# taha-kms/CLASSMATE-RAG

Hardware: AMD Instinct MI355X
Metric: hybrid queries/sec + recall@10 vs reference, 10M×768 chunks, 1/2/4/8 GPU (higher is better)
Workload: dtype fp32-accurate E5 (K10 f16x3 MFMA) + int8/f16/f64 dense + f64 BM25

## Files before the change

classmate-rag_amd/csrc/cm_dense_q8.inc:

```

#ifndef K1Q_RING
#define K1Q_RING 12
#endif
#ifndef K1Q_DBG
#define K1Q_DBG 0
#endif
constexpr int kQDbg = K1Q_DBG;
constexpr int kQRing = K1Q_RING;
constexpr int kQCap = 128;
#ifndef K1Q_RR
#define K1Q_RR 4096
#endif
#ifndef K1Q_RT
#define K1Q_RT 1024
#endif
constexpr int kQBand = K1Q_RR;
constexpr int kQBand2 = K1Q_RR / 2;
constexpr int kQRT = K1Q_RT, kQRW = K1Q_RT / 64;
constexpr int kQSel = 256;
constexpr int kQMeta = 4;
#ifndef K1Q_LDS
#define K1Q_LDS (160 * 1024)
#endif
#ifndef K1Q_LDS_SHARED
#define K1Q_LDS_SHARED (131 * 1024)
#endif
constexpr int q8_vm_after(int y, int z) {
  int n = 2 * (z - y);
  for (int x = y; x <= z; ++x) n += x % 6 == 0 ? 1 : 0;
  return n;
}

typedef int i32x4q __attribute__((ext_vector_type(4)));

__host__ __device__ inline void q8_ge(int k6, int &g, int &e) {
  g = k6 >> 4;
  e = k6 & 15;
}
__host__ __device__ inline int64_t q8_plane_off(int64_t row, int k, int ld) {
  const int64_t tile = row >> 6;
  const int rr = (int)(row & 63), rt = rr >> 4, j = rr & 15;
  const int c = k >> 7, kk = k & 127, kh = kk >> 6;
  int g, e;
  q8_ge(kk & 63, g, e);
  return (((tile * (ld >> 7) + c) * 8 + rt * 2 + kh) << 10) + ((g * 16 + j) << 4) + e;
}
__host__ __device__ inline int64_t q8_query_off(int64_t q, int k, int ld) {
  const int64_t qt = q >> 4;
  const int j = (int)(q & 15);
  const int c = k >> 7, kk = k & 127, kh = kk >> 6;
  int g, e;
  q8_ge(kk & 63, g, e);
  return (((qt * (ld >> 7) + c) * 2 + kh) << 10) + ((g * 16 + j) << 4) + e;
}

__device__ inline float block256_max(float v, float *red) {
  for (int o = 32; o > 0; o >>= 1) v = fmaxf(v, __shfl_xor(v, o));
  __syncthreads();
  if ((threadIdx.x & 63) == 0) red[threadIdx.x >> 6] = v;
  __syncthreads();
  return fmaxf(fmaxf(red[0], red[1]), fmaxf(red[2], red[3]));
}
__device__ inline double block256_sum(double v, double *red) {
  for (int o = 32; o > 0; o >>= 1) v += __shfl_xor(v, o);
  __syncthreads();
  if ((threadIdx.x & 63) == 0) red[threadIdx.x >> 6] = v;
  __syncthreads();
  return (red[0] + red[1]) + (red[2] + red[3]);
}

template <typename XN, typename PUT>
__device__ inline float3 q8_quantise(XN xn_of, PUT put, int ld) {
  __shared__ float redf[4];
  __shared__ double redd[4];
  float amax = 0.f;
  for (int c = threadIdx.x; c < ld; c += 256) amax = fmaxf(amax, fabsf(xn_of(c)));
  amax = block256_max(amax, redf);
  const float s = amax > 0.f ? amax / 127.f : 1.f;
  double er = 0.0, nr = 0.0;
  for (int c = threadIdx.x; c < ld; c += 256) {
    const float x = xn_of(c);
    const int q = max(-127, min(127, (int)rintf(x / s)));
    put(c, (int8_t)q);
    const double xt = (double)s * (double)q;
    er += ((double)x - xt) * ((double)x - xt);
    nr += xt * xt;
  }
  er = block256_sum(er, redd);
  nr = block256_sum(nr, redd);
  return make_float3(s, (float)(sqrt(er) * (1.0 + 1e-6)), (float)(sqrt(nr) * (1.0 + 1e-6)));
}

__host__ __device__ inline int64_t q8_group_of(int64_t row) { return (row >> 6) * 4 + ((row >> 2) & 3); }
__host__ __device__ inline int64_t q8_group_row(int64_t G, int i) {
  return (G >> 2) * 64 + 16 * (i >> 2) + 4 * (G & 3) + (i & 3);
}
__global__ void __launch_bounds__(256) dense_q8_group_kernel(const float *__restrict__ C, const float *__restrict__ invc,
                                                             const int64_t *__restrict__ groups, int64_t g0, int64_t ng,
                                                             int dim, int ld, int8_t *__restrict__ Xq,
                                                             float2 *__restrict__ rmeta, uint32_t *__restrict__ rnorm) {
  const int64_t gi = blockIdx.x;
  if (gi >= ng) return;
  const int64_t G = groups ? groups[gi] : g0 + gi;
  const int i = threadIdx.x >> 4, l = threadIdx.x & 15;
  const int64_t r = q8_group_row(G, i);
  const float inv = invc[r];
  const float *crow = C + r * ld;
  auto xn_of = [&](int c) { return c < dim ? crow[c] * inv : 0.f; };
  __shared__ float redf[4];
  float amax = 0.f;
  for (int c = l; c < ld; c += 16) amax = fmaxf(amax, fabsf(xn_of(c)));
  amax = block256_max(amax, redf);
  const float s = amax > 0.f ? amax / 127.f : 1.f;
  double er = 0.0, nr = 0.0;
  for (int c = l; c < ld; c += 16) {
    const float x = xn_of(c);
    const int q = max(-127, min(127, (int)rintf(x / s)));
    Xq[q8_plane_off(r, c, ld)] = (int8_t)q;
    const double xt = (double)s * (double)q;
    er += ((double)x - xt) * ((double)x - xt);
    nr += xt * xt;
  }
  for (int o = 8; o > 0; o >>= 1) {
    er += __shfl_xor(er, o);
    nr += __shfl_xor(nr, o);
  }
  if (l == 0) {
    rmeta[r] = make_float2(s, (float)(sqrt(er) * (1.0 + 1e-6)));
    atomicMax(&rnorm[2], __float_as_uint((float)(sqrt(nr) * (1.0 + 1e-6))));
  }
}

__global__ void __launch_bounds__(256) dense_prep_q8(const float *__restrict__ q, int nq, int dim, int ld,
                                                     int8_t *__restrict__ Qq, float4 *__restrict__ qsc,
                                                     const uint32_t *__restrict__ rnorm) {
  const int qi = blockIdx.x;
  const float *src = q + (int64_t)qi * dim;
  __shared__ double redd[4];
  double t = 0.0;
  float tf = 0.f;
  for (int i = threadIdx.x; i < dim; i += 256) {
    const float v = qi < nq ? src[i] : 0.f;
    tf += v * v;
  }
  __shared__ float redf[4];
  for (int o = 32; o > 0; o >>= 1) tf += __shfl_xor(tf, o);
  if ((threadIdx.x & 63) == 0) redf[threadIdx.x >> 6] = tf;
  __syncthreads();
  const float tt = (redf[0] + redf[1]) + (redf[2] + redf[3]);
  const float inv = 1.0f / (sqrtf(tt) + 1e-30f);
  auto xn_of = [&](int c) { return (qi < nq && c < dim) ? src[c] * inv : 0.f; };
  const float3 m = q8_quantise(xn_of, [&](int c, int8_t v) { Qq[q8_query_off(qi, c, ld)] = v; }, ld);
  for (int c = threadIdx.x; c < ld; c += 256) {
    const double x = (double)xn_of(c);
    t += x * x;
  }
  t = block256_sum(t, redd);
  if (threadIdx.x == 0) {
    const double nmax = (double)__uint_as_float(rnorm[2]);
    const float a = (float)(nmax * (double)m.y * (1.0 + 1e-6) + 4e-6);
    const float b = (float)(sqrt(t) * (1.0 + 1e-6));
    qsc[qi] = make_float4(m.x, a, b, sqrtf(tt));
  }
}

constexpr int kQDumpB = 96;
#ifndef K1Q_RING_FULL
#define K1Q_RING_FULL K1Q_RING
#endif
template <int LDS>
struct K1qLds {
  static constexpr int ring = LDS >= 160 * 1024 ? K1Q_RING_FULL : kQRing;
  static constexpr int stage_e = (LDS - ring * 8192 - kQMeta * 1024 - 1024) / (4 * kQDumpB);
  static constexpr int cnt_off = ring * 8192 + kQMeta * 1024 + 4 * stage_e * kQDumpB;
  static constexpr int total = cnt_off + 1024;
  static_assert(total <= 160 * 1024 && stage_e >= 64, "K1q LDS: ring + metadata + staging + counters");
};
constexpr int kQLds = K1qLds<K1Q_LDS>::total, kQLdsShared = K1qLds<K1Q_LDS_SHARED>::total;
template <int LDS = K1Q_LDS>
__global__ void __launch_bounds__(256, 1)
    dense_q8_scan_kernel(const int8_t *__restrict__ Xq, const float2 *__restrict__ rmeta,
                         const uint32_t *__restrict__ live, const uint32_t *__restrict__ allow, int64_t n_words,
                         const int8_t *__restrict__ Qq, const float4 *__restrict__ qsc, int nq,
                         const float *__restrict__ seed, int64_t rows_per_wg, int64_t rows_end, int n_wg,
                         uint64_t *__restrict__ out_keys, float *__restrict__ out_up,
                         uint32_t *__restrict__ out_cnt) {
  constexpr int KC = 6, QT = 4, PCS = 2, RING = K1qLds<LDS>::ring;
  constexpr int kQStageE = K1qLds<LDS>::stage_e, kQCntOff = K1qLds<LDS>::cnt_off;
  static_assert(RING > KC + 1, "the tile's row scales must be younger than every chunk the tile waits for");
  extern __shared__ __attribute__((aligned(16))) unsigned char lds[];
  const int tid = threadIdx.x, lane = tid & 63, g = lane >> 4, j = lane & 15;
  const int wave = __builtin_amdgcn_readfirstlane(tid >> 6);
  const int wg = blockIdx.x % n_wg, qp = blockIdx.x / n_wg;
  const int64_t r_begin = (int64_t)wg * rows_per_wg;
  const int64_t r_end = min(r_begin + rows_per_wg, rows_end);
  const int ntiles = r_begin < r_end ? (int)((r_end - r_begin) >> 6) : 0;
  const int total = ntiles * KC;
  const int qc0 = wave * 64;
  const int64_t qt0 = ((int64_t)qp * kBQPass + qc0) >> 4;
  i32x4q qf[KC][2][QT];
#pragma unroll
  for (int c = 0; c < KC; ++c)
#pragma unroll
    for (int kh = 0; kh < 2; ++kh)
#pragma unroll
      for (int qt = 0; qt < QT; ++qt)
        qf[c][kh][qt] = *reinterpret_cast<const i32x4q *>(Qq + ((((qt0 + qt) * KC + c) * 2 + kh) << 10) + lane * 16);
#pragma unroll
  for (int c = 0; c < KC; ++c)
#pragma unroll
    for (int kh = 0; kh < 2; ++kh)
#pragma unroll
      for (int qt = 0; qt < QT; ++qt) asm volatile("" : "+a"(qf[c][kh][qt]));
  float sq[QT], oaq[QT], aq[QT], bq[QT], sdq[QT];
#pragma unroll
  for (int qt = 0; qt < QT; ++qt) {
    const int qq = qp * kBQPass + qc0 + qt * 16 + j;
    const float4 v = qsc[qq];
    sq[qt] = v.x;
    aq[qt] = v.y;
    oaq[qt] = 1.0f - v.y;
    bq[qt] = v.z;
    sdq[qt] = qq < nq ? seed[qq] : -__builtin_inff();
  }
  __builtin_amdgcn_s_waitcnt(0x0F70);
  const __attribute__((address_space(1))) unsigned char *Xb = (const __attribute__((address_space(1))) unsigned char *)Xq;
  const int64_t cb = (r_begin >> 6) * KC;
  const uint32_t *allw = allow ? allow : live;
  unsigned char *meta = lds + RING * 8192;
  auto issue_meta = [&](int T) __attribute__((always_inline)) {
    const int Tc = min(T, ntiles - 1);
    const int64_t row0 = r_begin + (int64_t)Tc * 64;
    const unsigned char *src;
    if (wave == 2) {
      const int64_t wi = (row0 >> 5) + (lane & 1);
      const int64_t wc = wi < n_words ? wi : n_words - 1;
      src = reinterpret_cast<const unsigned char *>((lane & 2) ? allw + wc : live + wc);
    } else {
      src = reinterpret_cast<const unsigned char *>(rmeta + row0) + (wave & 1) * 256 + lane * 4;
    }
    __builtin_amdgcn_global_load_lds((const __attribute__((address_space(1))) void *)src,
                                     (__attribute__((address_space(3))) void *)(meta + (T % kQMeta) * 1024 + wave * 256),
                                     4, 0, 0);
  };
  auto issue_piece = [&](int gc, int i) __attribute__((always_inline)) {
    int gl = min(gc, total - 1);
    if (kQDbg & 8192) gl &= 15;
    const int o = 4 * i + wave;
    __builtin_amdgcn_global_load_lds(Xb + (((cb + gl) * 8 + o) << 10) + lane * 16,
                                     (__attribute__((address_space(3))) void *)(lds + (gc % RING) * 8192 + o * 1024),
                                     16, 0, kK1cAux);
  };
  auto issue = [&](int gc, bool tile_start) __attribute__((always_inline)) {
#pragma unroll
    for (int i = 0; i < PCS; ++i) issue_piece(gc, i);
    if (tile_start) issue_meta(gc / KC);
  };
  auto frag = [&](int gc, int rt, int kh) -> i32x4q {
    return *reinterpret_cast<const i32x4q *>(lds + (gc % RING) * 8192 + (rt * 2 + kh) * 1024 + lane * 16);
  };
  const uint32_t stg = (uint32_t)(uintptr_t)(const __attribute__((address_space(3))) unsigned char *)(
      lds + RING * 8192 + kQMeta * 1024 + wave * kQStageE * kQDumpB);
  const uint32_t cnt_lds = (uint32_t)(uintptr_t)(const __attribute__((address_space(3))) unsigned char *)(
      lds + kQCntOff + wave * 256);
  const int64_t qbuf0 = ((int64_t)qp * n_wg + wg) * kBQPass + qc0;
  uint32_t nst = 0, dbg_sink = 0;
  auto process = [&](uint32_t n) __attribute__((always_inline)) -> uint32_t {
    if (kQDbg & 16) return 0u;
    for (uint32_t e = lane; e < n; e += 64) {
      const uint32_t a0 = stg + e * kQDumpB;
      i32x4q h0, h1, av0, av1, av2, av3;
      asm volatile("ds_read_b128 %0, %6\n\t"
                   "ds_read_b128 %1, %6 offset:16\n\t"
                   "ds_read_b128 %2, %6 offset:32\n\t"
                   "ds_read_b128 %3, %6 offset:48\n\t"
                   "ds_read_b128 %4, %6 offset:64\n\t"
                   "ds_read_b128 %5, %6 offset:80\n\t"
                   "s_waitcnt lgkmcnt(0)"
                   : "=&v"(h0), "=&v"(h1), "=&v"(av0), "=&v"(av1), "=&v"(av2), "=&v"(av3)
                   : "v"(a0)
                   : "memory");
      const uint32_t ql = (uint32_t)h0[0] & 63u, live16 = (uint32_t)h0[0] >> 16;
      const int64_t rb = (int64_t)(uint32_t)h0[1];
      const float A = __int_as_float(h0[2]), B = __int_as_float(h0[3]);
      const float W = __int_as_float(h1[0]), sd = __int_as_float(h1[1]);
      const i32x4q av[4] = {av0, av1, av2, av3};
      uint32_t hm = 0;
#pragma unroll
      for (int i = 0; i < 16; ++i)
        hm |= (fmaf(-A, (float)av[i >> 2][i & 3], B) <= sd ? 1u : 0u) << i;
      hm &= live16;
      uint32_t slot;
      asm volatile("ds_add_rtn_u32 %0, %1, %2\n\ts_waitcnt lgkmcnt(0)"
                   : "=v"(slot) : "v"(cnt_lds + ql * 4), "v"((kQDbg & (2 | 32)) ? 0u : (uint32_t)__popc(hm))
                   : "memory");
      const int64_t ob = (qbuf0 + ql) * kQCap;
      if (kQDbg & 32) hm = 0;
      while (hm) {
        const int i = __builtin_ctz(hm);
        hm &= hm - 1u;
        int av_i;
        asm volatile("ds_read_b32 %0, %1\n\ts_waitcnt lgkmcnt(0)" : "=v"(av_i) : "v"(a0 + 32 + 4 * i) : "memory");
        if (slot < (uint32_t)kQCap && !(kQDbg & 2)) {
          const float lo = fmaf(-A, (float)av_i, B);
          const int64_t row = rb + 16 * (i >> 2) + (i & 3);
          out_keys[ob + slot] = ((uint64_t)f32_order(lo) << 32) | (uint64_t)(uint32_t)row;
          out_up[ob + slot] = lo + W;
        }
        ++slot;
      }
    }
    return 0u;
  };
  reinterpret_cast<uint32_t *>(lds + kQCntOff)[tid] = 0u;
  i32x4q acc[4][QT];
#pragma unroll
  for (int rt = 0; rt < 4; ++rt)
#pragma unroll
    for (int qt = 0; qt < QT; ++qt) acc[rt][qt] = i32x4q{0, 0, 0, 0};

  if (total > 0) {
#pragma unroll
    for (int p = 0; p < RING; ++p) issue(p, p % KC == 0);
    asm volatile("s_waitcnt vmcnt(%0)" ::"n"(q8_vm_after(0, RING - 1)) : "memory");
    __builtin_amdgcn_s_barrier();
    i32x4q xf[4][2];
#pragma unroll
    for (int rt = 0; rt < 2; ++rt)
#pragma unroll
      for (int kh = 0; kh < 2; ++kh) xf[rt][kh] = frag(0, rt, kh);
    constexpr int W0 = 16 - PCS - 2;
    const uint32_t meta_lds = (uint32_t)(uintptr_t)(const __attribute__((address_space(3))) unsigned char *)meta;
    int pm[QT];
    uint32_t eu = 0u, s_bits = 0u;
    i32x4q wdv;
    uint64_t ev[8];
    auto tail = [&](int m, int t) __attribute__((always_inline)) {
      const uint32_t mb = meta_lds + (t % kQMeta) * 1024;
      if (m == 0) {
        asm volatile("ds_read_b128 %0, %10 offset:512\n\t"
                     "ds_read_b32 %1, %11\n\t"
                     "ds_read2_b32 %2, %11 offset0:1 offset1:3\n\t"
                     "ds_read2_b32 %3, %11 offset0:5 offset1:7\n\t"
                     "ds_read2_b32 %4, %11 offset0:33 offset1:35\n\t"
                     "ds_read2_b32 %5, %11 offset0:37 offset1:39\n\t"
                     "ds_read2_b32 %6, %11 offset0:65 offset1:67\n\t"
                     "ds_read2_b32 %7, %11 offset0:69 offset1:71\n\t"
                     "ds_read2_b32 %8, %11 offset0:97 offset1:99\n\t"
                     "ds_read2_b32 %9, %11 offset0:101 offset1:103"
                     : "=&v"(wdv), "=&v"(s_bits), "=&v"(ev[0]), "=&v"(ev[1]), "=&v"(ev[2]), "=&v"(ev[3]),
                       "=&v"(ev[4]), "=&v"(ev[5]), "=&v"(ev[6]), "=&v"(ev[7])
                     : "v"(mb), "v"(mb + 32 * g)
                     : "memory");
      }
      if (m >= 3 && m <= 10) {
        const int q = (m - 3) >> 1;
        if (((m - 3) & 1) == 0) {
          pm[q] = max(max(acc[0][q][0], acc[0][q][1]), acc[0][q][2]);
          pm[q] = max(max(pm[q], acc[0][q][3]), acc[1][q][0]);
        } else {
          pm[q] = max(max(pm[q], acc[1][q][1]), acc[1][q][2]);
          pm[q] = max(pm[q], acc[1][q][3]);
        }
        asm volatile("" : "+v"(pm[q]));
      }
      if (m == 11) asm volatile("s_waitcnt lgkmcnt(0)" ::: "memory");
      if (m >= 11 && m <= 14) {
        const int k0 = 2 * (m - 11);
        eu = max(max(m == 11 ? 0u : eu, (uint32_t)ev[k0]), (uint32_t)(ev[k0] >> 32));
        eu = max(max(eu, (uint32_t)ev[k0 + 1]), (uint32_t)(ev[k0 + 1] >> 32));
        asm volatile("" : "+v"(eu));
      }
      if (m >= 12) {
        const int q = m - 12;
        pm[q] = max(max(pm[q], acc[2][q][0]), acc[2][q][1]);
        pm[q] = max(max(pm[q], acc[2][q][2]), acc[2][q][3]);
        asm volatile("" : "+v"(pm[q]));
      }
    };
#define K1Q_STEP(gcv, cc)                                                                                             \
  do {                                                                                                                \
    _Pragma("unroll") for (int m = 0; m < 16; ++m) {                                                                  \
      const int rt = m >> 3, kh = (m >> 2) & 1, qt = m & 3;                                                           \
      if (!(kQDbg & 4096))                                                                                            \
        acc[rt][qt] = __builtin_amdgcn_mfma_i32_16x16x64_i8(xf[rt][kh], qf[cc][kh][qt], acc[rt][qt], 0, 0, 0);        \
      __builtin_amdgcn_sched_barrier(0);                                                                              \
      if (m < 4) xf[2 + (m >> 1)][m & 1] = frag((gcv), 2 + (m >> 1), m & 1);                                          \
      if (m == W0) {                                                                                                  \
        asm volatile("s_waitcnt vmcnt(%0) lgkmcnt(0)" ::"n"(q8_vm_after((cc) + 1, (cc) + RING - 1)) : "memory");      \
        __builtin_amdgcn_s_barrier();                                                                                 \
      }                                                                                                               \
      if (!(kQDbg & 1024) && m > W0 && m <= W0 + PCS) issue_piece((gcv) + RING, m - W0 - 1);                          \
      if (!(kQDbg & 1024) && m == W0 + PCS + 1 && ((cc) + RING) % KC == 0) issue_meta(((gcv) + RING) / KC);           \
      __builtin_amdgcn_sched_barrier(0);                                                                              \
    }                                                                                                                 \
    _Pragma("unroll") for (int m = 0; m < 16; ++m) {                                                                  \
      const int rt = 2 + (m >> 3), kh = (m >> 2) & 1, qt = m & 3;                                                     \
      if (!(kQDbg & 4096))                                                                                            \
        acc[rt][qt] = __builtin_amdgcn_mfma_i32_16x16x64_i8(xf[rt][kh], qf[cc][kh][qt], acc[rt][qt], 0, 0, 0);        \
      __builtin_amdgcn_sched_barrier(0);                                                                              \
      if (m < 4) xf[m >> 1][m & 1] = frag((gcv) + 1, m >> 1, m & 1);                                                  \
      if ((cc) == KC - 1 && !(kQDbg & 128)) tail(m, t);                                                               \
      __builtin_amdgcn_sched_barrier(0);                                                                              \
    }                                                                                                                 \
  } while (0)
    for (int t = 0; t < ntiles; ++t) {
      const int64_t row0 = r_begin + (int64_t)t * 64;
      const int gc0 = t * KC;
      K1Q_STEP(gc0 + 0, 0);
      K1Q_STEP(gc0 + 1, 1);
      K1Q_STEP(gc0 + 2, 2);
      K1Q_STEP(gc0 + 3, 3);
      K1Q_STEP(gc0 + 4, 4);
      K1Q_STEP(gc0 + 5, 5);
      if (!(kQDbg & 128)) {
      const int64_t w0 = row0 >> 5;
      const uint32_t m0 = w0 < n_words ? ((uint32_t)wdv[0] & (uint32_t)wdv[2]) : 0u;
      const uint32_t m1 = w0 + 1 < n_words ? ((uint32_t)wdv[1] & (uint32_t)wdv[3]) : 0u;
      const bool full = (m0 & m1) == 0xffffffffu;
      const float S = __uint_as_float(s_bits);
      const float E = __uint_as_float(eu);
      int amax[QT];
      uint32_t live16 = 0xffffu;
      if (full) {
#pragma unroll
        for (int qt = 0; qt < QT; ++qt) {
          const int m = max(max(pm[qt], acc[3][qt][0]), acc[3][qt][1]);
          amax[qt] = max(max(m, acc[3][qt][2]), acc[3][qt][3]);
        }
      } else {
        live16 = lane_live16(((uint64_t)m1 << 32) | m0, g);
#pragma unroll
        for (int qt = 0; qt < QT; ++qt) {
          int m = INT32_MIN;
#pragma unroll
          for (int i = 0; i < 16; ++i) m = max(m, ((live16 >> i) & 1u) ? acc[i >> 2][qt][i & 3] : INT32_MIN);
          amax[qt] = m;
        }
      }
#pragma unroll
      for (int qt = 0; qt < QT; ++qt) {
        const float A = sq[qt] * S, B = fmaf(-bq[qt], E, oaq[qt]);
        const float W = 2.0f * fmaf(bq[qt], E, aq[qt]) + 1e-6f;
        const float lmin = fmaf(-A, (float)amax[qt], B);
        const bool pass = lmin <= sdq[qt] && amax[qt] != INT32_MIN;
        const uint64_t P = __ballot(pass);
        if (kQDbg & 64) {
          dbg_sink += (uint32_t)__popcll(P);
          continue;
        }
        if (P == 0) continue;
        const uint32_t np = (uint32_t)__popcll(P);
        if (nst + np > (uint32_t)kQStageE) nst = process(nst);
        if (pass) {
          const uint32_t pos = nst + __builtin_amdgcn_mbcnt_hi((uint32_t)(P >> 32), __builtin_amdgcn_mbcnt_lo((uint32_t)P, 0u));
          const uint32_t a = stg + pos * kQDumpB;
          const i32x4q h0 = {(int)((uint32_t)(qt * 16 + j) | (live16 << 16)), (int)(uint32_t)(row0 + 4 * g),
                             __float_as_int(A), __float_as_int(B)};
          const i32x4q h1 = {__float_as_int(W), __float_as_int(sdq[qt]), 0, 0};
          asm volatile("ds_write_b128 %0, %1\n\t"
                       "ds_write_b128 %0, %2 offset:16\n\t"
                       "ds_write_b128 %0, %3 offset:32\n\t"
                       "ds_write_b128 %0, %4 offset:48\n\t"
                       "ds_write_b128 %0, %5 offset:64\n\t"
                       "ds_write_b128 %0, %6 offset:80"
                       ::"v"(a), "v"(h0), "v"(h1), "v"(acc[0][qt]), "v"(acc[1][qt]), "v"(acc[2][qt]), "v"(acc[3][qt])
                       : "memory");
        }
        nst += np;
      }
      } else {
#pragma unroll
        for (int rt = 0; rt < 4; ++rt)
#pragma unroll
          for (int qt = 0; qt < QT; ++qt) dbg_sink += (uint32_t)acc[rt][qt][0];
      }
#pragma unroll
      for (int rt = 0; rt < 4; ++rt)
#pragma unroll
        for (int qt = 0; qt < QT; ++qt) acc[rt][qt] = i32x4q{0, 0, 0, 0};
    }
#undef K1Q_STEP
    asm volatile("s_waitcnt vmcnt(0)" ::: "memory");
    if (nst) nst = process(nst);
  }
  uint32_t c;
  asm volatile("ds_read_b32 %0, %1\n\ts_waitcnt lgkmcnt(0)" : "=v"(c) : "v"(cnt_lds + lane * 4) : "memory");
  if ((kQDbg & (64 | 128)) && dbg_sink == 0x7fffffffu) c = 0u;
  out_cnt[qbuf0 + lane] = c;
}

#ifndef K1QS_RING
#define K1QS_RING 4
#endif
constexpr int cgcd(int a, int b) { return b == 0 ? a : cgcd(b, a % b); }
template <int QT, int R>
__global__ void __launch_bounds__(256, 1)
    dense_q8_stream_kernel(const int8_t *__restrict__ Xq, const float2 *__restrict__ rmeta,
                           const uint32_t *__restrict__ live, const uint32_t *__restrict__ allow, int64_t n_words,
                           const int8_t *__restrict__ Qq, const float4 *__restrict__ qsc, int nq,
                           const float *__restrict__ seed, int64_t rows_per_vg, int64_t rows_end, int n_vg,
                           uint64_t *__restrict__ out_keys, float *__restrict__ out_up,
                           uint32_t *__restrict__ out_cnt) {
  constexpr int KC = 6;
  constexpr int TU = R / cgcd(R, KC);
  const int lane = threadIdx.x & 63, g = lane >> 4, j = lane & 15;
  const int wave = __builtin_amdgcn_readfirstlane(threadIdx.x >> 6);
  const int vg = blockIdx.x * 4 + wave;
  if (vg >= n_vg) return;
  const int64_t r_begin = (int64_t)vg * rows_per_vg;
  const int64_t r_end = min(r_begin + rows_per_vg, rows_end);
  const int ntiles = r_begin < r_end ? (int)((r_end - r_begin) >> 6) : 0;
  const int total = ntiles * KC;

  i32x4q qf[KC][2][QT];
#pragma unroll
  for (int c = 0; c < KC; ++c)
#pragma unroll
    for (int kh = 0; kh < 2; ++kh)
#pragma unroll
      for (int qt = 0; qt < QT; ++qt)
        qf[c][kh][qt] = *reinterpret_cast<const i32x4q *>(Qq + (((qt * KC + c) * 2 + kh) << 10) + lane * 16);
#pragma unroll
  for (int c = 0; c < KC; ++c)
#pragma unroll
    for (int kh = 0; kh < 2; ++kh)
#pragma unroll
      for (int qt = 0; qt < QT; ++qt) asm volatile("" : "+a"(qf[c][kh][qt]));
  float sq[QT], oaq[QT], aq[QT], bq[QT], sdq[QT];
  uint32_t qcnt[QT];
#pragma unroll
  for (int qt = 0; qt < QT; ++qt) {
    const int qq = qt * 16 + j;
    const float4 v = qsc[qq];
    sq[qt] = v.x;
    aq[qt] = v.y;
    oaq[qt] = 1.0f - v.y;
    bq[qt] = v.z;
    sdq[qt] = qq < nq ? seed[qq] : -__builtin_inff();
    qcnt[qt] = 0u;
  }
  i32x4q acc[4][QT];
#pragma unroll
  for (int rt = 0; rt < 4; ++rt)
#pragma unroll
    for (int qt = 0; qt < QT; ++qt) acc[rt][qt] = i32x4q{0, 0, 0, 0};

  if (total > 0) {
    const i32x4q *Xv = reinterpret_cast<const i32x4q *>(Xq);
    const int64_t chunk0 = (r_begin >> 6) * KC;
    i32x4q xb[R][8];
    auto load = [&](i32x4q (&b)[8], int gc) __attribute__((always_inline)) {
      const int gl = min(gc, total - 1);
      const i32x4q *p = Xv + (chunk0 + gl) * 512 + lane;
#pragma unroll
      for (int i = 0; i < 8; ++i) b[i] = __builtin_nontemporal_load(p + i * 64);
    };
#pragma unroll
    for (int p = 0; p < R - 1; ++p) load(xb[p], p);
    for (int t = 0; t < ntiles; t += TU) {
#pragma unroll
      for (int u = 0; u < TU; ++u) {
        const int tt = t + u;
        const int tc = min(tt, ntiles - 1);
        const int64_t row0 = r_begin + (int64_t)tc * 64;
        f32x4 mr[4][2];
#pragma unroll
        for (int rt = 0; rt < 4; ++rt)
#pragma unroll
          for (int h = 0; h < 2; ++h)
            mr[rt][h] = __builtin_nontemporal_load(reinterpret_cast<const f32x4 *>(rmeta + row0 + 16 * rt + 4 * g) + h);
        uint32_t lw, aw;
        bool w_ok;
        {
          const int64_t wi = (row0 >> 5) + (lane & 1);
          w_ok = wi < n_words;
          const int64_t wc = w_ok ? wi : n_words - 1;
          lw = __builtin_nontemporal_load(live + wc);
          aw = __builtin_nontemporal_load((allow ? allow : live) + wc);
        }
#pragma unroll
        for (int c = 0; c < KC; ++c) {
          const int lc = u * KC + c;
          load(xb[(lc + R - 1) % R], tt * KC + c + R - 1);
          __builtin_amdgcn_sched_barrier(0);
          const int s = lc % R;
#pragma unroll
          for (int rt = 0; rt < 4; ++rt)
#pragma unroll
            for (int kh = 0; kh < 2; ++kh)
#pragma unroll
              for (int qt = 0; qt < QT; ++qt)
                acc[rt][qt] = __builtin_amdgcn_mfma_i32_16x16x64_i8(xb[s][rt * 2 + kh], qf[c][kh][qt], acc[rt][qt], 0, 0, 0);
          __builtin_amdgcn_sched_barrier(0);
        }
        if (tt < ntiles) {
          const uint32_t tw = w_ok ? (lw & aw) : 0u;
          const uint32_t b0 = (uint32_t)__builtin_amdgcn_readlane((int)tw, 0);
          const uint32_t b1 = (uint32_t)__builtin_amdgcn_readlane((int)tw, 1);
          const bool full = (b0 & b1) == 0xffffffffu;
          const uint32_t live16 = full ? 0xffffu : lane_live16(((uint64_t)b1 << 32) | b0, g);
          const float S = mr[0][0][0];
          float E = 0.f;
#pragma unroll
          for (int rt = 0; rt < 4; ++rt)
#pragma unroll
            for (int h = 0; h < 2; ++h) E = fmaxf(E, fmaxf(mr[rt][h][1], mr[rt][h][3]));
#pragma unroll
          for (int qt = 0; qt < QT; ++qt) {
            int amax;
            if (full) {
              amax = acc[0][qt][0];
#pragma unroll
              for (int i = 1; i < 16; ++i) amax = max(amax, acc[i >> 2][qt][i & 3]);
            } else {
              amax = INT32_MIN;
#pragma unroll
              for (int i = 0; i < 16; ++i) amax = max(amax, ((live16 >> i) & 1u) ? acc[i >> 2][qt][i & 3] : INT32_MIN);
            }
            const float A = sq[qt] * S, B = fmaf(-bq[qt], E, oaq[qt]);
            const float W = 2.0f * fmaf(bq[qt], E, aq[qt]) + 1e-6f;
            const bool pass = amax != INT32_MIN && fmaf(-A, (float)amax, B) <= sdq[qt];
            if (__ballot(pass) == 0) continue;
            uint32_t hm = 0;
            if (pass) {
#pragma unroll
              for (int i = 0; i < 16; ++i) hm |= (fmaf(-A, (float)acc[i >> 2][qt][i & 3], B) <= sdq[qt] ? 1u : 0u) << i;
              hm &= live16;
            }
            const int c = __popc(hm);
            const int c0 = __shfl(c, j), c1 = __shfl(c, 16 + j), c2 = __shfl(c, 32 + j), c3 = __shfl(c, 48 + j);
            uint32_t slot = qcnt[qt] + (uint32_t)((g > 0 ? c0 : 0) + (g > 1 ? c1 : 0) + (g > 2 ? c2 : 0));
            qcnt[qt] += (uint32_t)(c0 + c1 + c2 + c3);
            if (hm) {
              const int64_t ob = ((int64_t)vg * kSQ + qt * 16 + j) * kQCap;
#pragma unroll
              for (int i = 0; i < 16; ++i) {
                if ((hm >> i) & 1u) {
                  if (slot < (uint32_t)kQCap) {
                    const float lo = fmaf(-A, (float)acc[i >> 2][qt][i & 3], B);
                    const int64_t row = row0 + 16 * (i >> 2) + 4 * g + (i & 3);
                    out_keys[ob + slot] = ((uint64_t)f32_order(lo) << 32) | (uint64_t)(uint32_t)row;
                    out_up[ob + slot] = lo + W;
                  }
                  ++slot;
                }
              }
            }
          }
        }
#pragma unroll
        for (int rt = 0; rt < 4; ++rt)
#pragma unroll
          for (int qt = 0; qt < QT; ++qt) acc[rt][qt] = i32x4q{0, 0, 0, 0};
      }
    }
  }
  if (g == 0) {
#pragma unroll
    for (int qt = 0; qt < QT; ++qt) out_cnt[(int64_t)vg * kSQ + qt * 16 + j] = qcnt[qt];
  }
}

template <typename V>
__device__ inline uint32_t block_select_fn(V val, int n, int kk, uint32_t *hist) {
  __shared__ uint32_t s_prefix, s_rem;
  if (threadIdx.x == 0) {
    s_prefix = 0;
    s_rem = (uint32_t)kk;
  }
  for (int shift = 24; shift >= 0; shift -= 8) {
    for (int b = threadIdx.x; b < 256; b += blockDim.x) hist[b] = 0;
    __syncthreads();
    const uint32_t prefix = s_prefix;
    const uint32_t hmask = shift == 24 ? 0u : (0xffffffffu << (shift + 8));
    for (int i = threadIdx.x; i < n; i += blockDim.x) {
      const uint32_t x = val(i);
      if ((x & hmask) == (prefix & hmask)) atomicAdd(&hist[(x >> shift) & 255u], 1u);
    }
    __syncthreads();
    if (threadIdx.x < 64) {
      const int l = threadIdx.x;
      const uint32_t h0 = hist[4 * l], h1 = hist[4 * l + 1], h2 = hist[4 * l + 2], h3 = hist[4 * l + 3];
      const uint32_t sum = h0 + h1 + h2 + h3;
      uint32_t incl = sum;
#pragma unroll
      for (int o = 1; o < 64; o <<= 1) {
        const uint32_t v = __shfl_up(incl, o);
        if (l >= o) incl += v;
      }
      const uint32_t rem = s_rem, excl = incl - sum;
      if (excl <= rem && rem < incl) {
        uint32_t r = rem - excl, b = 4u * l;
        if (r >= h0) {
          r -= h0;
          ++b;
          if (r >= h1) {
            r -= h1;
            ++b;
            if (r >= h2) {
              r -= h2;
              ++b;
            }
          }
        }
        s_prefix = prefix | (b << shift);
        s_rem = r;
      }
    }
    __syncthreads();
  }
  return s_prefix;
}

constexpr int kQGather = K1Q_RR;
constexpr int kQRows = 8;
constexpr int kQRerankLds = kQGather * 12;
__global__ void __launch_bounds__(kQRT) dense_rerank_q8_kernel(
    const uint64_t *__restrict__ keys, const float *__restrict__ ups, const uint32_t *__restrict__ cnts, int n_wg,
    int qs, int k, int nq, const float *__restrict__ C, int ld, int dim, const float *__restrict__ q,
    const float4 *__restrict__ qsc, const _Float16 *__restrict__ Xh, const _Float16 *__restrict__ Qh,
    const float *__restrict__ qnorm, const float *__restrict__ row_norms, float *__restrict__ out_dist,
    int64_t *__restrict__ out_row, int32_t *__restrict__ fb_mask, int32_t *__restrict__ fb_count,
    uint32_t *__restrict__ fb_bound) {
  const int qi = blockIdx.x;
  if (qi >= nq) return;
  const int tid = threadIdx.x, lane = tid & 63, wave = tid >> 6;
  const int qp = qi / qs, ql = qi - qp * qs;
  extern __shared__ __attribute__((aligned(16))) unsigned char dyn[];
  uint64_t *g_key = reinterpret_cast<uint64_t *>(dyn);
  uint32_t *g_up = reinterpret_cast<uint32_t *>(dyn + kQGather * 8);
  __shared__ uint32_t s_off[2049];
  __shared__ uint32_t hist[256];
  __shared__ float s_q[768];
  __shared__ int s_flag, s_total, s_band;
  __shared__ uint64_t s_sel[kQSel];
  __shared__ int s_nsel;
  static_assert(kQBand * 4 <= kQGather * 4 && kQBand * 4 <= kQGather * 4 && kQBand2 * 8 <= kQGather * 4, "K1q re-rank LDS");
  uint32_t *s_rows = g_up;
  uint64_t *s_ex = g_key;
  if (tid == 0) {
    s_flag = 0;
    s_band = 0;
    s_nsel = 0;
  }
  __syncthreads();
  if (wave == 0) {
    uint32_t run = 0;
    for (int b0 = 0; b0 < n_wg; b0 += 64) {
      const int b = b0 + lane;
      uint32_t c = b < n_wg ? cnts[((int64_t)qp * n_wg + b) * qs + ql] : 0u;
      if (c > (uint32_t)kQCap) {
        s_flag = 1;
        c = kQCap;
      }
      uint32_t incl = c;
      for (int o = 1; o < 64; o <<= 1) {
        const uint32_t v = __shfl_up(incl, o);
        if (lane >= o) incl += v;
      }
      if (b < n_wg) s_off[b] = run + incl - c;
      run += __shfl(incl, 63);
    }
    if (lane == 0) {
      s_off[n_wg] = run;
      s_total = (int)run;
    }
  }
  __syncthreads();
  const int total = s_total;
  auto slot_of = [&](int jj) -> int64_t {
    int lo = 0, hi = n_wg - 1;
    while (lo < hi) {
      const int mid = (lo + hi + 1) >> 1;
      if (s_off[mid] <= (uint32_t)jj) lo = mid;
      else hi = mid - 1;
    }
    return (((int64_t)qp * n_wg + lo) * qs + ql) * kQCap + (jj - s_off[lo]);
  };
  const bool gathered = total <= kQGather;
  if (gathered) {
#pragma unroll 4
    for (int jj = tid; jj < total; jj += kQRT) {
      const int64_t sl = slot_of(jj);
      g_key[jj] = keys[sl];
      g_up[jj] = f32_order(ups[sl]);
    }
  }
  for (int i = tid; i < 768; i += kQRT) s_q[i] = i < dim ? q[(int64_t)qi * dim + i] : 0.f;
  __syncthreads();
  auto key_at = [&](int jj) -> uint64_t { return gathered ? g_key[jj] : keys[slot_of(jj)]; };
  auto up_at = [&](int jj) -> uint32_t { return gathered ? g_up[jj] : f32_order(ups[slot_of(jj)]); };
  uint32_t tkey = 0xffffffffu;
  if (total >= k) tkey = block_select_fn(up_at, total, k - 1, hist);
  if (s_flag) {
    if (tid == 0) {
      fb_mask[qi] = 2;
      fb_bound[qi] = tkey;
      atomicAdd(fb_count, 1);
    }
    return;
  }
  for (int jj = tid; jj < total; jj += kQRT) {
    const uint64_t key = key_at(jj);
    if (tkey == 0xffffffffu || (uint32_t)(key >> 32) <= tkey) {
      const int p = atomicAdd(&s_band, 1);
      if (p < kQBand) s_rows[p] = (uint32_t)key;
    }
  }
  __syncthreads();
  const int band = s_band;
  if (band > kQBand) {
    if (tid == 0) {
      fb_mask[qi] = 2;
      fb_bound[qi] = tkey;
      atomicAdd(fb_count, 1);
    }
    return;
  }
  if (tid == 0) {
    fb_mask[qi] = 0;
    fb_bound[qi] = 0u;
  }
  const uint32_t *band_rows = s_rows;
  int band2 = band;
  if (Xh != nullptr) {
  float *s_dh = reinterpret_cast<float *>(dyn);
  uint32_t *s_rows2 = reinterpret_cast<uint32_t *>(dyn + kQGather * 4);
  const float Eh = coarse_err(qnorm, qi, row_norms, dim);
  {
    typedef _Float16 h2 __attribute__((ext_vector_type(2)));
    const int hl = lane & 31, hh = lane >> 5;
    f16x8 qv[3];
    int kof[3];
#pragma unroll
    for (int u = 0; u < 3; ++u) {
      const int pc = hl + 32 * u;
      kof[u] = 64 * (pc >> 3) + 32 * ((pc >> 2) & 1) + 8 * (pc & 3);
      qv[u] = *reinterpret_cast<const f16x8 *>(Qh + (int64_t)qi * ld + kof[u]);
    }
    constexpr int RP = 4;
    for (int c0 = wave * 2 * RP; c0 < band; c0 += kQRW * 2 * RP) {
      f16x8 xv[RP][3];
#pragma unroll
      for (int rp = 0; rp < RP; ++rp) {
        const int c = min(c0 + 2 * rp + hh, band - 1);
        const int64_t row = s_rows[c];
        const int64_t tile = row >> 6;
        const int rr = (int)(row & 63), rt = rr >> 4, jj = rr & 15;
#pragma unroll
        for (int u = 0; u < 3; ++u) {
          const int pc = hl + 32 * u, cch = pc >> 3, sb = (pc >> 2) & 1, gg = pc & 3;
          xv[rp][u] = *reinterpret_cast<const f16x8 *>(
              Xh + ((((tile * (ld >> 6) + cch) * 8 + rt * 2 + sb) << 9) + ((jj * 4 + gg) << 3)));
        }
      }
#pragma unroll
      for (int rp = 0; rp < RP; ++rp) {
        float acc = 0.f;
#pragma unroll
        for (int u = 0; u < 3; ++u)
#pragma unroll
          for (int e = 0; e < 8; e += 2)
            acc = __builtin_amdgcn_fdot2(h2{xv[rp][u][e], xv[rp][u][e + 1]}, h2{qv[u][e], qv[u][e + 1]}, acc, false);
#pragma unroll
        for (int o = 16; o > 0; o >>= 1) acc += __shfl_xor(acc, o);
        const int c = c0 + 2 * rp + hh;
        if (hl == 0 && c < band) s_dh[c] = 1.0f - acc;
      }
    }
  }
  __syncthreads();
  {
    const uint32_t kth_h = band >= k ? block_select_fn([&](int i) { return f32_order(s_dh[i] + Eh); }, band, k - 1, hist)
                                     : 0xffffffffu;
    if (tid == 0) s_band = 0;
    __syncthreads();
    for (int c = tid; c < band; c += kQRT)
      if (kth_h == 0xffffffffu || f32_order(s_dh[c] - Eh) <= kth_h) s_rows2[atomicAdd(&s_band, 1)] = s_rows[c];
    __syncthreads();
  }
  band2 = s_band;
  band_rows = s_rows2;
  if (band2 > kQBand2) {
    if (tid == 0) {
      fb_mask[qi] = 2;
      fb_bound[qi] = tkey;
      atomicAdd(fb_count, 1);
    }
    return;
  }
  }
  const double qnrm = (double)qsc[qi].w;
  constexpr int M = 12;
  for (int c0 = wave * kQRows; c0 < band2; c0 += kQRW * kQRows) {
    float x[kQRows][M];
    uint32_t rows[kQRows];
#pragma unroll
    for (int r = 0; r < kQRows; ++r) {
      const int c = min(c0 + r, band2 - 1);
      rows[r] = band_rows[c];
      const float *cr = C + (int64_t)rows[r] * ld + lane;
#pragma unroll
      for (int m = 0; m < M; ++m) x[r][m] = cr[64 * m];
    }
    double dq[kQRows], dc[kQRows];
#pragma unroll
    for (int r = 0; r < kQRows; ++r) {
      dq[r] = 0.0;
      dc[r] = 0.0;
#pragma unroll
      for (int m = 0; m < M; ++m) {
        const double xv = (double)x[r][m];
        dq[r] += xv * (double)s_q[lane + 64 * m];
        dc[r] += xv * xv;
      }
    }
    for (int o = 32; o > 0; o >>= 1) {
#pragma unroll
      for (int r = 0; r < kQRows; ++r) {
        dq[r] += __shfl_xor(dq[r], o);
        dc[r] += __shfl_xor(dc[r], o);
      }
    }
    if (lane == 0) {
#pragma unroll
      for (int r = 0; r < kQRows; ++r)
        if (c0 + r < band2) {
          const float dist = (float)(1.0 - dq[r] / ((sqrt(dc[r]) + 1e-30) * (qnrm + 1e-30)));
          s_ex[c0 + r] = ((uint64_t)f32_order(dist) << 32) | rows[r];
        }
    }
  }
  __syncthreads();
  const uint32_t thi = band2 > k ? block_select_fn([&](int i) { return (uint32_t)(s_ex[i] >> 32); }, band2, k - 1, hist)
                                : 0xffffffffu;
  for (int c = tid; c < band2; c += kQRT) {
    const uint64_t key = s_ex[c];
    if ((uint32_t)(key >> 32) <= thi) {
      const int p = atomicAdd(&s_nsel, 1);
      if (p < kQSel) s_sel[p] = key;
    }
  }
  __syncthreads();
  const int nsel = s_nsel;
  const uint64_t *cand = nsel <= kQSel ? s_sel : s_ex;
  const int ncand = nsel <= kQSel ? nsel : band2;
  for (int c = tid; c < ncand; c += kQRT) {
    const uint64_t key = cand[c];
    int rank = 0;
    for (int i = 0; i < ncand; ++i) rank += cand[i] < key ? 1 : 0;
    if (rank < k) {
      out_dist[(int64_t)qi * k + rank] = f32_unorder((uint32_t)(key >> 32));
      out_row[(int64_t)qi * k + rank] = (int64_t)(uint32_t)key;
    }
  }
  for (int i = band2 + tid; i < k; i += kQRT) {
    out_dist[(int64_t)qi * k + i] = 0.f;
    out_row[(int64_t)qi * k + i] = -1;
  }
}

constexpr int kWideSlots = 16;
constexpr int kWideCap = 1 << 16;
constexpr int kWideThreads = 1024;
constexpr int kWideOvf = 64;
__global__ void __launch_bounds__(kWideThreads) dense_rerank_wide_kernel(
    const uint64_t *__restrict__ keys, const uint32_t *__restrict__ cnts, int n_wg, int qs, int k, int nq,
    const float *__restrict__ C, int ld, int dim, const float *__restrict__ q, const float4 *__restrict__ qsc,
    const _Float16 *__restrict__ Xh, const _Float16 *__restrict__ Qh, const float *__restrict__ qnorm,
    const float *__restrict__ row_norms, const int8_t *__restrict__ Xq, const float2 *__restrict__ rmeta,
    const int8_t *__restrict__ Qq, const uint32_t *__restrict__ live, const uint32_t *__restrict__ allow,
    int64_t n_words, int64_t rows_per_wg, int64_t rows_end,
    float *__restrict__ out_dist, int64_t *__restrict__ out_row, int32_t *__restrict__ fb_mask,
    int32_t *__restrict__ fb_count, const uint32_t *__restrict__ fb_bound, int32_t *__restrict__ wide_ctr,
    uint32_t *__restrict__ wide_rows, uint64_t *__restrict__ wide_keys) {
  const int qi = blockIdx.x;
  if (qi >= nq || *fb_count == 0 || fb_mask[qi] != 2) return;
  const int tid = threadIdx.x, lane = tid & 63, wave = tid >> 6;
  constexpr int NW = kWideThreads / 64;
  const int qp = qi / qs, ql = qi - qp * qs;
  __shared__ uint32_t s_off[2049];
  __shared__ uint32_t hist[256];
  __shared__ float s_q[768];
  __shared__ uint64_t s_sel[kQSel];
  __shared__ int s_ovf[kWideOvf];
  __shared__ int s_slot, s_n, s_nsel, s_total, s_novf;
  if (tid == 0) {
    s_slot = 0;
    s_n = 0;
    s_nsel = 0;
    s_novf = 0;
  }
  __syncthreads();
  {
    int before = 0;
    for (int j = tid; j < qi; j += kWideThreads) before += fb_bound[j] != 0u ? 1 : 0;
    if (before) atomicAdd(&s_slot, before);
  }
  if (wave == 0) {
    uint32_t run = 0;
    for (int b0 = 0; b0 < n_wg; b0 += 64) {
      const int b = b0 + lane;
      uint32_t c = b < n_wg ? cnts[((int64_t)qp * n_wg + b) * qs + ql] : 0u;
      if (c > (uint32_t)kQCap) {
        const int o = atomicAdd(&s_novf, 1);
        if (o < kWideOvf) s_ovf[o] = b;
        c = 0;
      }
      uint32_t incl = c;
      for (int o = 1; o < 64; o <<= 1) {
        const uint32_t v = __shfl_up(incl, o);
        if (lane >= o) incl += v;
      }
      if (b < n_wg) s_off[b] = run + incl - c;
      run += __shfl(incl, 63);
    }
    if (lane == 0) {
      s_off[n_wg] = run;
      s_total = (int)run;
    }
  }
  for (int i = tid; i < 768; i += kWideThreads) s_q[i] = i < dim ? q[(int64_t)qi * dim + i] : 0.f;
  __syncthreads();
  const int slot = s_slot;
  const int novf = s_novf;
  if (slot >= kWideSlots || novf > kWideOvf) {
    if (tid == 0) fb_mask[qi] = 1;
    return;
  }
  uint32_t *rows = wide_rows + (int64_t)slot * kWideCap;
  uint64_t *wk = wide_keys + (int64_t)slot * kWideCap;
  const uint32_t tkey = fb_bound[qi];
  const int total = s_total;
  for (int jj = tid; jj < total; jj += kWideThreads) {
    int lo = 0, hi = n_wg - 1;
    while (lo < hi) {
      const int mid = (lo + hi + 1) >> 1;
      if (s_off[mid] <= (uint32_t)jj) lo = mid;
      else hi = mid - 1;
    }
    const uint64_t key = keys[(((int64_t)qp * n_wg + lo) * qs + ql) * kQCap + (jj - s_off[lo])];
    if ((uint32_t)(key >> 32) <= tkey) {
      const int p = atomicAdd(&s_n, 1);
      if (p < kWideCap) rows[p] = (uint32_t)key;
    }
  }
  if (novf > 0 && Xh == nullptr) {
    const float4 qs4 = qsc[qi];
    const int64_t qt = qi >> 4;
    const int jq = qi & 15;
    const int c = lane >> 3, kh = (lane >> 2) & 1, gq = lane & 3;
    i32x4q qv = {0, 0, 0, 0};
    if (lane < 48)
      qv = *reinterpret_cast<const i32x4q *>(Qq + ((((qt * (ld >> 7) + c) * 2 + kh) << 10) + ((gq * 16 + jq) << 4)));
    for (int g = 0; g < novf; ++g) {
      const int64_t r0 = (int64_t)s_ovf[g] * rows_per_wg, r1 = min(r0 + rows_per_wg, rows_end);
      for (int64_t row = r0 + wave; row < r1; row += NW) {
        if ((row >> 5) >= n_words) break;
        const uint32_t lw = live[row >> 5] & (allow ? allow[row >> 5] : 0xffffffffu);
        if (!((lw >> (row & 31)) & 1u)) continue;
        const int64_t tile = row >> 6;
        const int rr = (int)(row & 63), rt = rr >> 4, jj = rr & 15;
        int acc = 0;
        if (lane < 48) {
          const i32x4q xv = *reinterpret_cast<const i32x4q *>(
              Xq + ((((tile * (ld >> 7) + c) * 8 + rt * 2 + kh) << 10) + ((gq * 16 + jj) << 4)));
#pragma unroll
          for (int e = 0; e < 4; ++e) acc = __builtin_amdgcn_sdot4(xv[e], qv[e], acc, false);
        }
        for (int o = 32; o > 0; o >>= 1) acc += __shfl_xor(acc, o);
        const float2 m = rmeta[row];
        const float lo = fmaf(-(qs4.x * m.x), (float)acc, fmaf(-qs4.z, m.y, 1.0f - qs4.y));
        if (lane == 0 && f32_order(lo) <= tkey) {
          const int p = atomicAdd(&s_n, 1);
          if (p < kWideCap) rows[p] = (uint32_t)row;
        }
      }
    }
  }
  if (novf > 0 && Xh != nullptr) {
    typedef _Float16 h2 __attribute__((ext_vector_type(2)));
    const float Eh = coarse_err(qnorm, qi, row_norms, dim);
    const int hl = lane & 31, hh = lane >> 5;
    f16x8 qv[3];
#pragma unroll
    for (int u = 0; u < 3; ++u) {
      const int pc = hl + 32 * u;
      qv[u] = *reinterpret_cast<const f16x8 *>(Qh + (int64_t)qi * ld + 64 * (pc >> 3) + 32 * ((pc >> 2) & 1) + 8 * (pc & 3));
    }
    for (int g = 0; g < novf; ++g) {
      const int64_t r0 = (int64_t)s_ovf[g] * rows_per_wg, r1 = min(r0 + rows_per_wg, rows_end);
      for (int64_t row = r0 + 2 * wave + hh; row < r1; row += 2 * NW) {
        if ((row >> 5) >= n_words) break;
        const uint32_t lw = live[row >> 5] & (allow ? allow[row >> 5] : 0xffffffffu);
        if (!((lw >> (row & 31)) & 1u)) continue;
        const int64_t tile = row >> 6;
        const int rr = (int)(row & 63), rt = rr >> 4, jj = rr & 15;
        float acc = 0.f;
#pragma unroll
        for (int u = 0; u < 3; ++u) {
          const int pc = hl + 32 * u, cch = pc >> 3, sb = (pc >> 2) & 1, gg = pc & 3;
          const f16x8 xv = *reinterpret_cast<const f16x8 *>(
              Xh + ((((tile * (ld >> 6) + cch) * 8 + rt * 2 + sb) << 9) + ((jj * 4 + gg) << 3)));
#pragma unroll
          for (int e = 0; e < 8; e += 2)
            acc = __builtin_amdgcn_fdot2(h2{xv[e], xv[e + 1]}, h2{qv[u][e], qv[u][e + 1]}, acc, false);
        }
#pragma unroll
        for (int o = 16; o > 0; o >>= 1) acc += __shfl_xor(acc, o, 32);
        if (hl == 0 && f32_order(1.0f - acc - Eh) <= tkey) {
          const int p = atomicAdd(&s_n, 1);
          if (p < kWideCap) rows[p] = (uint32_t)row;
        }
      }
    }
  }
  __syncthreads();
  const int n = s_n;
  if (n > kWideCap) {
    if (tid == 0) fb_mask[qi] = 1;
    return;
  }
  const double qnrm = (double)qsc[qi].w;
  constexpr int M = 12, WR = 4;
  for (int c0 = wave * WR; c0 < n; c0 += NW * WR) {
    float x[WR][M];
    uint32_t rr[WR];
#pragma unroll
    for (int r = 0; r < WR; ++r) {
      const int c = min(c0 + r, n - 1);
      rr[r] = rows[c];
      const float *cr = C + (int64_t)rr[r] * ld + lane;
#pragma unroll
      for (int m = 0; m < M; ++m) x[r][m] = cr[64 * m];
    }
    double dq[WR], dc[WR];
#pragma unroll
    for (int r = 0; r < WR; ++r) {
      dq[r] = 0.0;
      dc[r] = 0.0;
#pragma unroll
      for (int m = 0; m < M; ++m) {
        const double xv = (double)x[r][m];
        dq[r] += xv * (double)s_q[lane + 64 * m];
        dc[r] += xv * xv;
      }
    }
    for (int o = 32; o > 0; o >>= 1) {
#pragma unroll
      for (int r = 0; r < WR; ++r) {
        dq[r] += __shfl_xor(dq[r], o);
        dc[r] += __shfl_xor(dc[r], o);
      }
    }
    if (lane == 0) {
#pragma unroll
      for (int r = 0; r < WR; ++r)
        if (c0 + r < n) {
          const float dist = (float)(1.0 - dq[r] / ((sqrt(dc[r]) + 1e-30) * (qnrm + 1e-30)));
          wk[c0 + r] = ((uint64_t)f32_order(dist) << 32) | rr[r];
        }
    }
  }
  __threadfence_block();
  __syncthreads();
  const uint32_t thi = n > k ? block_select_fn([&](int i) { return (uint32_t)(wk[i] >> 32); }, n, k - 1, hist)
                             : 0xffffffffu;
  for (int c = tid; c < n; c += kWideThreads) {
    const uint64_t key = wk[c];
    if ((uint32_t)(key >> 32) <= thi) {
      const int p = atomicAdd(&s_nsel, 1);
      if (p < kQSel) s_sel[p] = key;
    }
  }
  __syncthreads();
  const int nsel = s_nsel;
  if (nsel > kQSel) {
    if (tid == 0) fb_mask[qi] = 1;
    return;
  }
  for (int c = tid; c < nsel; c += kWideThreads) {
    const uint64_t key = s_sel[c];
    int rank = 0;
    for (int i = 0; i < nsel; ++i) rank += s_sel[i] < key ? 1 : 0;
    if (rank < k) {
      out_dist[(int64_t)qi * k + rank] = f32_unorder((uint32_t)(key >> 32));
      out_row[(int64_t)qi * k + rank] = (int64_t)(uint32_t)key;
    }
  }
  for (int i = n + tid; i < k; i += kWideThreads) {
    out_dist[(int64_t)qi * k + i] = 0.f;
    out_row[(int64_t)qi * k + i] = -1;
  }
  if (tid == 0) {
    fb_mask[qi] = 0;
    atomicSub(fb_count, 1);
    atomicAdd(wide_ctr + 1, 1);
  }
}
```

Baseline: 34860.

## Tighten rerank band bound with exact f64 pilot scoring of top-k candidates

Before building the rerank band, the kernel exactly scores in f64 the candidates whose upper bound is within the k-th bound. It then uses their k-th exact distance as a tighter cutoff (bkey) for admitting rows into the band. This is meant to shrink the band and the f16 plus f64 rerank work, and to reduce fallbacks caused by band overflow. The cost is an extra pass of global row loads, a block select and several barriers per query. The duplicated f64 distance code is also factored into a shared template helper.

```diff
diff --git a/classmate-rag_amd/csrc/cm_dense_q8.inc b/classmate-rag_amd/csrc/cm_dense_q8.inc
--- a/classmate-rag_amd/csrc/cm_dense_q8.inc
+++ b/classmate-rag_amd/csrc/cm_dense_q8.inc
@@ -713,8 +713,43 @@
   return s_prefix;
 }
 
+template <int R>
+__device__ inline void rows_dist_f64(const float *__restrict__ C, int ld, const uint32_t (&rows)[R], const float *sq,
+                                     double qnrm, int lane, float (&dist)[R]) {
+  constexpr int M = 12;
+  float x[R][M];
+#pragma unroll
+  for (int r = 0; r < R; ++r) {
+    const float *cr = C + (int64_t)rows[r] * ld + lane;
+#pragma unroll
+    for (int m = 0; m < M; ++m) x[r][m] = cr[64 * m];
+  }
+  double dq[R], dc[R];
+#pragma unroll
+  for (int r = 0; r < R; ++r) {
+    dq[r] = 0.0;
+    dc[r] = 0.0;
+#pragma unroll
+    for (int m = 0; m < M; ++m) {
+      const double xv = (double)x[r][m];
+      dq[r] += xv * (double)sq[lane + 64 * m];
+      dc[r] += xv * xv;
+    }
+  }
+  for (int o = 32; o > 0; o >>= 1) {
+#pragma unroll
+    for (int r = 0; r < R; ++r) {
+      dq[r] += __shfl_xor(dq[r], o);
+      dc[r] += __shfl_xor(dc[r], o);
+    }
+  }
+#pragma unroll
+  for (int r = 0; r < R; ++r) dist[r] = (float)(1.0 - dq[r] / ((sqrt(dc[r]) + 1e-30) * (qnrm + 1e-30)));
+}
+
 constexpr int kQGather = K1Q_RR;
 constexpr int kQRows = 8;
+constexpr int kQPilotRows = kQRW >= 16 ? 2 : kQRW >= 8 ? 4 : 8;
 constexpr int kQRerankLds = kQGather * 12;
 __global__ void __launch_bounds__(kQRT) dense_rerank_q8_kernel(
     const uint64_t *__restrict__ keys, const float *__restrict__ ups, const uint32_t *__restrict__ cnts, int n_wg,
@@ -801,9 +836,39 @@
     }
     return;
   }
+  const double qnrm = (double)qsc[qi].w;
+  uint32_t bkey = tkey;
+  if (total >= k) {
+    for (int jj = tid; jj < total; jj += kQRT)
+      if (up_at(jj) <= tkey) {
+        const int p = atomicAdd(&s_nsel, 1);
+        if (p < kQSel) s_sel[p] = key_at(jj);
+      }
+    __syncthreads();
+    const int np = s_nsel;
+    if (np <= kQSel) {
+      for (int c0 = wave * kQPilotRows; c0 < np; c0 += kQRW * kQPilotRows) {
+        uint32_t rows[kQPilotRows];
+        float dist[kQPilotRows];
+#pragma unroll
+        for (int r = 0; r < kQPilotRows; ++r) rows[r] = (uint32_t)s_sel[c0 + r < np ? c0 + r : c0];
+        rows_dist_f64<kQPilotRows>(C, ld, rows, s_q, qnrm, lane, dist);
+        if (lane == 0) {
+#pragma unroll
+          for (int r = 0; r < kQPilotRows; ++r)
+            if (c0 + r < np) s_sel[c0 + r] = ((uint64_t)f32_order(dist[r]) << 32) | rows[r];
+        }
+      }
+      __syncthreads();
+      const uint32_t pkey = block_select_fn([&](int i) { return (uint32_t)(s_sel[i] >> 32); }, np, k - 1, hist);
+      bkey = min(tkey, pkey);
+    }
+    __syncthreads();
+    if (tid == 0) s_nsel = 0;
+  }
   for (int jj = tid; jj < total; jj += kQRT) {
     const uint64_t key = key_at(jj);
-    if (tkey == 0xffffffffu || (uint32_t)(key >> 32) <= tkey) {
+    if (total < k || (uint32_t)(key >> 32) <= bkey) {
       const int p = atomicAdd(&s_band, 1);
       if (p < kQBand) s_rows[p] = (uint32_t)key;
     }
@@ -813,7 +878,7 @@
   if (band > kQBand) {
     if (tid == 0) {
       fb_mask[qi] = 2;
-      fb_bound[qi] = tkey;
+      fb_bound[qi] = bkey;
       atomicAdd(fb_count, 1);
     }
     return;
@@ -885,51 +950,22 @@
   if (band2 > kQBand2) {
     if (tid == 0) {
       fb_mask[qi] = 2;
-      fb_bound[qi] = tkey;
+      fb_bound[qi] = bkey;
       atomicAdd(fb_count, 1);
     }
     return;
   }
   }
-  const double qnrm = (double)qsc[qi].w;
-  constexpr int M = 12;
   for (int c0 = wave * kQRows; c0 < band2; c0 += kQRW * kQRows) {
-    float x[kQRows][M];
     uint32_t rows[kQRows];
-#pragma unroll
-    for (int r = 0; r < kQRows; ++r) {
-      const int c = min(c0 + r, band2 - 1);
-      rows[r] = band_rows[c];
-      const float *cr = C + (int64_t)rows[r] * ld + lane;
-#pragma unroll
-      for (int m = 0; m < M; ++m) x[r][m] = cr[64 * m];
-    }
-    double dq[kQRows], dc[kQRows];
-#pragma unroll
-    for (int r = 0; r < kQRows; ++r) {
-      dq[r] = 0.0;
-      dc[r] = 0.0;
-#pragma unroll
-      for (int m = 0; m < M; ++m) {
-        const double xv = (double)x[r][m];
-        dq[r] += xv * (double)s_q[lane + 64 * m];
-        dc[r] += xv * xv;
-      }
-    }
-    for (int o = 32; o > 0; o >>= 1) {
-#pragma unroll
-      for (int r = 0; r < kQRows; ++r) {
-        dq[r] += __shfl_xor(dq[r], o);
-        dc[r] += __shfl_xor(dc[r], o);
-      }
-    }
+    float dist[kQRows];
+#pragma unroll
+    for (int r = 0; r < kQRows; ++r) rows[r] = band_rows[min(c0 + r, band2 - 1)];
+    rows_dist_f64<kQRows>(C, ld, rows, s_q, qnrm, lane, dist);
     if (lane == 0) {
 #pragma unroll
       for (int r = 0; r < kQRows; ++r)
-        if (c0 + r < band2) {
-          const float dist = (float)(1.0 - dq[r] / ((sqrt(dc[r]) + 1e-30) * (qnrm + 1e-30)));
-          s_ex[c0 + r] = ((uint64_t)f32_order(dist) << 32) | rows[r];
-        }
+        if (c0 + r < band2) s_ex[c0 + r] = ((uint64_t)f32_order(dist[r]) << 32) | rows[r];
     }
   }
   __syncthreads();
@@ -1123,44 +1159,17 @@
     return;
   }
   const double qnrm = (double)qsc[qi].w;
-  constexpr int M = 12, WR = 4;
+  constexpr int WR = 4;
   for (int c0 = wave * WR; c0 < n; c0 += NW * WR) {
-    float x[WR][M];
     uint32_t rr[WR];
-#pragma unroll
-    for (int r = 0; r < WR; ++r) {
-      const int c = min(c0 + r, n - 1);
-      rr[r] = rows[c];
-      const float *cr = C + (int64_t)rr[r] * ld + lane;
-#pragma unroll
-      for (int m = 0; m < M; ++m) x[r][m] = cr[64 * m];
-    }
-    double dq[WR], dc[WR];
-#pragma unroll
-    for (int r = 0; r < WR; ++r) {
-      dq[r] = 0.0;
-      dc[r] = 0.0;
-#pragma unroll
-      for (int m = 0; m < M; ++m) {
-        const double xv = (double)x[r][m];
-        dq[r] += xv * (double)s_q[lane + 64 * m];
-        dc[r] += xv * xv;
-      }
-    }
-    for (int o = 32; o > 0; o >>= 1) {
-#pragma unroll
-      for (int r = 0; r < WR; ++r) {
-        dq[r] += __shfl_xor(dq[r], o);
-        dc[r] += __shfl_xor(dc[r], o);
-      }
-    }
+    float dist[WR];
+#pragma unroll
+    for (int r = 0; r < WR; ++r) rr[r] = rows[min(c0 + r, n - 1)];
+    rows_dist_f64<WR>(C, ld, rr, s_q, qnrm, lane, dist);
     if (lane == 0) {
 #pragma unroll
       for (int r = 0; r < WR; ++r)
-        if (c0 + r < n) {
-          const float dist = (float)(1.0 - dq[r] / ((sqrt(dc[r]) + 1e-30) * (qnrm + 1e-30)));
-          wk[c0 + r] = ((uint64_t)f32_order(dist) << 32) | rr[r];
-        }
+        if (c0 + r < n) wk[c0 + r] = ((uint64_t)f32_order(dist[r]) << 32) | rr[r];
     }
   }
   __threadfence_block();
```

Result: faster. 35520 (median of 6 runs) (+1.9%).
